# Indra-jith/failure-aware-vision

Hardware: AMD Instinct MI355X
Metric: frames/sec, ResNet-50 MC-Dropout T=30 224x224 batch=256 (higher is better)
Workload: dtype bf16; 1 GPU; BASELINE configs[2]: ResNet-50 v1.5 + MC-Dropout T=30 (all_blocks, p=0.10), 224x224x3 fp32 frames with Gaussian noise severity 3, batch 256 per GPU, synthetic frames and seeded synthetic weights; frames_per_gpu=256, global_batch=256, mc_samples=30, dropout_policy=all_blocks, inputs=resident in HBM before the timed region (H2D excluded), parallelism=batch sharded, 1 process per GPU, all-gather of (label, confidence)

## Files before the change

### failure_aware_vision_amd/_lib.py

```python
from __future__ import annotations

import ctypes as C
import os

_HERE = os.path.dirname(os.path.abspath(__file__))
LIB_PATH = os.environ.get("FAV_LIB_PATH") or os.path.join(_HERE, "lib", "libfav_hip.so")

FAV_OK = 0
STATUS_NAMES = {0: "FAV_OK", 1: "FAV_ERR_INVALID_ARG", 2: "FAV_ERR_BAD_BLOB", 3: "FAV_ERR_NO_WEIGHTS",
                4: "FAV_ERR_HIP", 5: "FAV_ERR_NO_DEVICE", 6: "FAV_ERR_UNSUPPORTED"}
LAYOUT_NHWC_U8, LAYOUT_NHWC_F32 = 0, 1
ARCH_RESNET18_CIFAR, ARCH_RESNET50, ARCH_VIT_B16, ARCH_VIT_TINY = 0, 1, 2, 3
CONF_MAX_SOFTMAX, CONF_ENTROPY, CONF_MUTUAL_INFO = 0, 1, 2
MATH_BF16, MATH_F32_EXACT = 0, 1
K_STEM, K_CONV, K_MAXPOOL, K_AVGPOOL, K_DROPOUT, K_HEAD, K_COUNT = 0, 1, 2, 3, 4, 5, 6
KERNEL_CLASS_NAMES = ("stem_im2col", "conv_igemm", "maxpool", "avgpool", "entry_dropout", "head")


class FavConfig(C.Structure):
    _fields_ = [
        ("struct_size", C.c_uint32), ("device", C.c_int32), ("arch", C.c_int32), ("num_classes", C.c_int32),
        ("in_h", C.c_int32), ("in_w", C.c_int32), ("max_batch", C.c_int32),
        ("mean", C.c_float * 3), ("stdev", C.c_float * 3),
        ("n_samples", C.c_int32), ("site_mask", C.c_uint32), ("dropout_p", C.c_float), ("seed", C.c_uint64),
# ... 54 lines not shown


class FavProfile(C.Structure):
    _fields_ = [("ms", C.c_double * K_COUNT), ("flops", C.c_double * K_COUNT), ("bytes", C.c_double * K_COUNT),
                ("launches", C.c_int64 * K_COUNT)]


class FavOpProfile(C.Structure):
    _fields_ = [("op_index", C.c_int32), ("kind", C.c_int32), ("H", C.c_int32), ("W", C.c_int32), ("Cin", C.c_int32),
                ("Ho", C.c_int32), ("Wo", C.c_int32), ("Cout", C.c_int32), ("kh", C.c_int32), ("kw", C.c_int32),
                ("stride", C.c_int32), ("reserved", C.c_int32), ("ms", C.c_double), ("flops", C.c_double),
                ("bytes", C.c_double), ("launches", C.c_int64)]


_SIGNATURES = {
    "fav_abi_version": (C.c_int32, []),
    "fav_default_config": (None, [C.POINTER(FavConfig), C.c_int32]),
    "fav_create": (C.c_int, [C.POINTER(FavConfig), C.POINTER(C.c_void_p)]),
    "fav_load_weights": (C.c_int, [C.c_void_p, C.c_void_p, C.c_size_t]),
    "fav_load_member_weights": (C.c_int, [C.c_void_p, C.c_int32, C.c_void_p, C.c_size_t]),
    "fav_destroy": (None, [C.c_void_p]),
    "fav_check_blob": (C.c_int, [C.c_void_p, C.c_size_t, C.c_char_p, C.c_size_t]),
    "fav_plan_schedule": (C.c_int, [C.POINTER(FavConfig), C.c_int32, C.c_char_p, C.c_size_t]),
    "fav_last_error": (C.c_char_p, [C.c_void_p]),
    "fav_classify": (C.c_int, [C.c_void_p, C.c_void_p, C.c_int32, C.c_int32, C.c_void_p, C.c_void_p, C.c_void_p]),
    "fav_classify_ex": (C.c_int, [C.c_void_p, C.c_void_p, C.c_int32, C.c_int32, C.c_int64, C.c_void_p, C.c_void_p,
                                  C.c_void_p, C.c_void_p, C.c_void_p]),
    "fav_classify_records": (C.c_int, [C.c_void_p, C.c_void_p, C.c_int32, C.c_int32, C.c_int64, C.c_void_p, C.c_void_p,
                                      C.c_void_p, C.c_void_p]),
    "fav_classify_uncertainty": (C.c_int, [C.c_void_p, C.c_void_p, C.c_int32, C.c_int32, C.c_int64, C.c_void_p, C.c_void_p,
                                          C.c_void_p, C.c_void_p]),
    "fav_classify_sets": (C.c_int, [C.c_void_p, C.c_void_p, C.c_int32, C.c_int32, C.c_int64, C.POINTER(FavConformal),
                                    C.c_void_p, C.c_void_p, C.c_void_p, C.c_void_p]),
    "fav_conformal_scores": (C.c_int, [C.c_void_p, C.c_void_p, C.c_int32, C.c_int32, C.c_int64, C.POINTER(FavConformal),
                                       C.c_void_p, C.c_void_p, C.c_void_p]),
    "fav_classify_sweep": (C.c_int, [C.c_void_p, C.c_void_p, C.c_int32, C.c_int32, C.c_int64, C.c_void_p, C.POINTER(C.c_float),
                                     C.c_int32, C.c_void_p, C.c_void_p]),
    "fav_set_temperature": (C.c_int, [C.c_void_p, C.c_float]),
    "fav_set_tau": (C.c_int, [C.c_void_p, C.c_float]),
    "fav_classify_host": (C.c_int, [C.c_void_p, C.c_void_p, C.c_int32, C.c_int32, C.c_int64, C.c_void_p, C.c_void_p,
                                    C.c_void_p, C.c_void_p]),
    "fav_get_logits": (C.c_int, [C.c_void_p, C.c_void_p, C.POINTER(C.c_int32), C.POINTER(C.c_int32), C.c_void_p]),
    "fav_set_profiling": (C.c_int, [C.c_void_p, C.c_int32]),
    "fav_get_profile": (C.c_int, [C.c_void_p, C.POINTER(FavProfile), C.c_int32]),
    "fav_get_op_profile": (C.c_int, [C.c_void_p, C.POINTER(FavOpProfile), C.c_int32, C.POINTER(C.c_int32)]),
    "fav_op_conv2d": (C.c_int, [C.POINTER(FavConvDesc), C.c_void_p]),
    "fav_op_bottleneck_tail": (C.c_int, [C.POINTER(FavTailDesc), C.c_void_p]),
    "fav_op_linear_streamk": (C.c_int, [C.POINTER(FavLinearDesc), C.c_void_p]),
    "fav_op_stem_im2col": (C.c_int, [C.c_void_p, C.c_int32, C.c_int32, C.c_int32, C.c_int32, C.c_int32, C.c_int32,
                                     C.c_int32, C.c_int32, C.c_int32, C.POINTER(C.c_float), C.POINTER(C.c_float),
                                     C.c_void_p, C.c_void_p]),
    "fav_op_stem_pool": (C.c_int, [C.c_void_p, C.c_int32, C.c_int32, C.c_int32, C.c_int32, C.c_void_p, C.c_void_p, C.c_void_p, C.c_void_p, C.c_void_p, C.c_void_p]),
    "fav_op_maxpool3x3s2": (C.c_int, [C.c_void_p, C.c_void_p, C.c_int32, C.c_int32, C.c_int32, C.c_int32, C.c_void_p]),
    "fav_op_avgpool": (C.c_int, [C.c_void_p, C.c_void_p, C.c_int32, C.c_int32, C.c_int32, C.POINTER(FavDropoutDesc),
                                 C.c_void_p]),
    "fav_op_entry_dropout": (C.c_int, [C.c_void_p, C.c_void_p, C.c_int64, C.c_int32, C.POINTER(FavDropoutDesc),
                                       C.c_void_p]),
    "fav_op_entry_reduce": (C.c_int, [C.c_void_p, C.c_void_p, C.c_void_p, C.c_void_p, C.c_void_p, C.c_int32, C.c_int32, C.c_int32,
                                      C.c_int32, C.POINTER(FavDropoutDesc), C.c_void_p]),
    "fav_op_layernorm": (C.c_int, [C.c_void_p, C.c_int64, C.c_void_p, C.c_void_p, C.c_void_p, C.c_int64, C.c_int32, C.c_float,
                                   C.c_void_p]),
    "fav_op_attention": (C.c_int, [C.c_void_p, C.c_void_p, C.c_int32, C.c_int32, C.c_int32, C.c_int32, C.c_int32, C.c_void_p]),
    "fav_op_vit_assemble": (C.c_int, [C.c_void_p, C.c_void_p, C.c_void_p, C.c_int32, C.c_int32, C.c_int32, C.c_void_p]),
    "fav_op_head": (C.c_int, [C.c_void_p, C.c_int32, C.c_int32, C.c_int32, C.c_int32, C.c_float, C.c_int32, C.c_float,
                              C.c_void_p, C.c_void_p, C.c_void_p, C.c_void_p, C.c_void_p]),
    "fav_op_head_uncertainty": (C.c_int, [C.c_void_p, C.c_int32, C.c_int32, C.c_int32, C.c_int32, C.c_float, C.c_int32,
                                          C.c_float, C.c_void_p, C.c_void_p, C.c_void_p, C.c_void_p]),
    "fav_op_head_sets": (C.c_int, [C.c_void_p, C.c_int32, C.c_int32, C.c_int32, C.c_int32, C.c_float, C.c_int32, C.c_float,
                                   C.c_int64, C.POINTER(FavConformal), C.c_void_p, C.c_void_p, C.c_void_p, C.c_void_p,
                                   C.c_void_p, C.c_void_p]),
# ... 36 lines not shown
```

### failure_aware_vision_amd/csrc/fav.hip

```cpp
#include <hip/hip_runtime.h>

#include <algorithm>
#include <atomic>
#include <cmath>
#include <cstdarg>
#include <cstdio>
#include <cstdlib>
#include <cstring>
#include <string>
#include <vector>

#include "../../include/fav.h"
#include "fav_kernels.hpp"
#include "fav_plan.hpp"

using namespace fav_plan;

namespace {

thread_local std::string g_create_error;

std::string fmt(const char* f, ...) {
    char buf[512];
    va_list ap;
// ... 331 lines not shown
    } while (0)
#define FAV_LAUNCH_BIG(MODE_)                                                                                     \
    do {                                                                                                          \
        const int pp = (int)FAV_KNOB("FAV_CONV_PP", 1);                                                           \
        if (d.relu == 2) {                                                                                        \
            if (epi && pp && MODE_ == 0) hipLaunchKernelGGL((conv_igemm_kernel<256, 256, 64, 2, 0, 2, 0, 1, 1, true>), grid, dim3(512), 0, s, p); \
            else if (epi) hipLaunchKernelGGL((conv_igemm_kernel<256, 256, 64, 2, MODE_, 2, 0, 1, 0, true>), grid, dim3(512), 0, s, p);    \
            else hipLaunchKernelGGL((conv_igemm_kernel<256, 256, 64, 2, MODE_, 2, 0, 0, 0, true>), grid, dim3(512), 0, s, p);        \
        } else if (epi && pp && MODE_ == 0) hipLaunchKernelGGL((conv_igemm_kernel<256, 256, 64, 2, 0, 2, 0, 1, 1>), grid, dim3(512), 0, s, p); \
        else if (epi) hipLaunchKernelGGL((conv_igemm_kernel<256, 256, 64, 2, MODE_, 2, 0, 1>), grid, dim3(512), 0, s, p);    \
        else hipLaunchKernelGGL((conv_igemm_kernel<256, 256, 64, 2, MODE_, 2, 0, 0>), grid, dim3(512), 0, s, p);        \
    } while (0)
    if (big) {
        if (d.math_mode == FAV_MATH_BF16) FAV_LAUNCH_BIG(0); else FAV_LAUNCH_BIG(1);
    } else if (d.math_mode == FAV_MATH_BF16) FAV_LAUNCH_MODE(0); else FAV_LAUNCH_MODE(1);
#undef FAV_LAUNCH_BIG
#undef FAV_LAUNCH_MODE
#undef FAV_LAUNCH
    dbg_report(tiles, BM, BN, BK);
    return nullptr;
}


const char* launch_tail(fav_handle* h, const fav_tail_desc& d, const Group& G, hipStream_t s) {
    const bool has3x3 = d.wb != nullptr;
    const int nred = d.wa ? d.Nred : 0;
    TailGeom g;
    if (!tail_geometry(d.Cmid, nred, has3x3, d.W, &g)) return "bottleneck tail: unsupported shape";
    const long long M = (long long)d.n_frames * d.H * d.W;
    if (M <= 0 || M > 0x7fffffffLL) return "bottleneck tail: row count out of range";
    TailParams p;
    p.t1 = (const uint16_t*)d.x; p.wb = (const uint16_t*)d.wb; p.bias_b = d.bias_b;
    p.wc = (const uint16_t*)d.wc; p.bias_c = d.bias_c; p.res = (const uint16_t*)d.res; p.y = (uint16_t*)d.y;
    p.wa = (const uint16_t*)d.wa; p.bias_a = d.bias_a; p.t1n = (uint16_t*)d.t1n;
    p.H = d.H; p.W = d.W; p.HW = d.H * d.W; p.M = (int)M;
    p.in_W = d.W; p.in_HW = p.HW; p.in_stride = 1;
    p.rega_bytes = g.rega_bytes;
    p.bias_b_off = g.bias_b_off; p.bias_ca_off = g.bias_ca_off; p.wa_off0 = g.wa_off0; p.wa_off1 = g.wa_off1; p.zero_off = g.zero_off;
    p.drop = make_drop(&d.drop);
    p.div_hw = fastdiv_make((uint32_t)p.HW);
    p.div_w = fastdiv_make((uint32_t)d.W);
    if (p.drop.site >= 0 && (p.drop.v0 < 0 || p.drop.v0 + d.n_frames > 0x7fffffffLL)) return "bottleneck tail: virtual frame index out of range";
    p.g_t1 = G.x; p.g_res = G.res; p.g_y = G.y; p.g_t1n = G.y2;
    p.g_wb = G.wb; p.g_bb = G.bb; p.g_wc = G.w; p.g_bc = G.b; p.g_wa = G.wa; p.g_ba = G.ba;
    p.site_e = d.entry_site;
    p.rs_T = 0; p.rs_tps = 0;
    if (d.res_entry) {
        if (!(d.Cmid == 64 && nred == 64 && has3x3) || p.drop.site < 0 || d.entry_site < 0 || !d.res)
            return "bottleneck tail: res_entry needs Cmid = Nred = 64 with the 3x3 and both dropout sites";
        if ((double)p.drop.n_img * p.HW * 4.0 * d.Cmid * 2.0 >= 2147483647.0) return "bottleneck tail: cached tensor too large for 32-bit offsets";
    }
    const int cmid = d.Cmid, cout = 4 * cmid;
    const double flops = 2.0 * (double)M * ((has3x3 ? 9.0 * cmid * cmid : 0.0) + (double)cmid * cout + (double)cout * nred) * G.n;
    const double res_rows = d.res_entry ? (double)std::min<long long>(d.n_frames, p.drop.n_img) * p.HW : (double)M;
    const double bytes = 2.0 * ((double)M * (cmid + 1.0 * cout + nred) + res_rows * cout + (has3x3 ? 9.0 * cmid * cmid : 0.0) + (double)cmid * cout + (double)cout * nred) * G.n;
    Prof pr(h, s, FAV_K_CONV, flops, bytes);
    { const int lds_pad = (int)FAV_KNOB("FAV_TAIL_LDS_PAD", 0); if (g.lds_bytes + lds_pad <= 160 * 1024) g.lds_bytes += lds_pad; }
    const int bm = g.rp * g.nw;
    const long long nblocks = (M + bm - 1) / bm;
    dim3 grid((unsigned)nblocks, G.n);
    p.dbg = nullptr;
    const bool dbg_on = FAV_KNOB("FAV_CONV_DBG", 0) != 0;
    if (dbg_on && !h) { (void)hipMalloc((void**)&p.dbg, (size_t)nblocks * 128); (void)hipMemset(p.dbg, 0, (size_t)nblocks * 128); }
    auto dbg_report = [&]() {
        if (!p.dbg) return;
        (void)hipStreamSynchronize(s);
        std::vector<unsigned long long> t((size_t)nblocks * 16);
        (void)hipMemcpy(t.data(), p.dbg, t.size() * 8, hipMemcpyDeviceToHost);
        (void)hipFree(p.dbg);
        if (const char* dump = fav_knob_str("FAV_CONV_DBG_DUMP")) {
            if (FILE* f = fopen(dump, "ab")) { const long long hdr[2] = {nblocks, cmid * 1000 + nred}; fwrite(hdr, 8, 2, f); fwrite(t.data(), 8, t.size(), f); fclose(f); }
        }
        unsigned long long lo = ~0ull, hi = 0;
        double ph[5] = {0, 0, 0, 0, 0};
        double cy[5] = {0, 0, 0, 0, 0};
        double cz[3] = {0, 0, 0};
        for (long long i = 0; i < nblocks; ++i) {
            lo = std::min(lo, t[i * 16]); hi = std::max(hi, t[i * 16 + 5]);
// ... 16 lines not shown
        static DeviceFlags attr_set;                                                                                  \
        if (!attr_set.test_current()) {                                                                               \
            if (hipFuncSetAttribute((const void*)bottleneck_tail_kernel<CMID_, NRED_, H3_, NS_, NW_, WC2_>,           \
                                    hipFuncAttributeMaxDynamicSharedMemorySize, 160 * 1024) != hipSuccess)            \
                return "bottleneck tail: cannot reserve LDS";                                                         \
            attr_set.set_current();                                                                                   \
        }                                                                                                             \
        hipLaunchKernelGGL((bottleneck_tail_kernel<CMID_, NRED_, H3_, NS_, NW_, WC2_>), grid, dim3(NW_ * 64), g.lds_bytes, s, p, g.patch_bytes); \
        dbg_report();                                                                                                 \
        return nullptr;                                                                                               \
    } while (0)
#define FAV_TAIL_W(CMID_, NRED_, H3_, NS_, NW_) do { if (g.wc2) FAV_TAIL(CMID_, NRED_, H3_, NS_, NW_, true); else FAV_TAIL(CMID_, NRED_, H3_, NS_, NW_, false); } while (0)
#define FAV_TAIL_N(CMID_, NRED_, H3_, NS_) FAV_TAIL_W(CMID_, NRED_, H3_, NS_, 4)
    if (d.res_entry) {
        const bool sample_minor = FAV_KNOB("FAV_ENTRY_RES_ORDER", 1) != 0;
        const long long sample_rows = (long long)p.drop.n_img * p.HW;
        if (sample_minor && p.drop.v0 % p.drop.n_img == 0 && d.n_frames % p.drop.n_img == 0 && sample_rows % bm == 0) {
            p.rs_T = d.n_frames / p.drop.n_img;
            p.rs_tps = (int)(sample_rows / bm);
        }
        static DeviceFlags attr_set;
        auto k0 = bottleneck_tail_kernel<64, 64, true, 3, 4, false, 32, 0, true, true, true>;
        auto k1 = bottleneck_tail_kernel<64, 64, true, 3, 4, true, 32, 0, true, true, true>;
        if (!attr_set.test_current()) {
            if (hipFuncSetAttribute((const void*)k0, hipFuncAttributeMaxDynamicSharedMemorySize, 160 * 1024) != hipSuccess ||
                hipFuncSetAttribute((const void*)k1, hipFuncAttributeMaxDynamicSharedMemorySize, 160 * 1024) != hipSuccess)
                return "bottleneck tail: cannot reserve LDS";
            attr_set.set_current();
        }
        if (g.wc2) hipLaunchKernelGGL(k1, grid, dim3(256), g.lds_bytes, s, p, g.patch_bytes);
        else hipLaunchKernelGGL(k0, grid, dim3(256), g.lds_bytes, s, p, g.patch_bytes);
        dbg_report();
        return nullptr;
    }
    if (cmid == 64) {
        if (has3x3) { if (nred == 0) FAV_TAIL_N(64, 0, true, 3); if (nred == 64) FAV_TAIL_N(64, 64, true, 3); if (nred == 128) FAV_TAIL_N(64, 128, true, 3); }
        else { if (nred == 0) FAV_TAIL_N(64, 0, false, 3); if (nred == 64) FAV_TAIL_N(64, 64, false, 3); if (nred == 128) FAV_TAIL_N(64, 128, false, 3); }
    } else if (cmid == 128) {
        if (has3x3) { if (nred == 0) FAV_TAIL_W(128, 0, true, 2, 8); if (nred == 128) FAV_TAIL_W(128, 128, true, 2, 8); }
        else { if (nred == 0) FAV_TAIL_W(128, 0, false, 2, 8); if (nred == 128) FAV_TAIL_W(128, 128, false, 2, 8); }
    } else if (cmid == 512) {
        FAV_TAIL(512, 0, false, 2, 8, true);
    } else if (nred == 0 && has3x3) {
        FAV_TAIL(256, 0, true, 2, 8, true);
    } else if (nred == 0) {
        FAV_TAIL_W(256, 0, false, 2, 4);
// ... 487 lines not shown
                case OP_CONV: {
                    const LayerShape& L = h->plan.layers[o.layer];
                    fav_conv_desc d;
                    d.x = buf(o.in, o); d.w = LW(o.layer); d.bias = LB(o.layer); d.res = buf(o.res, o); d.y = buf(o.out, o);
                    d.n_frames = cn; d.H = o.H; d.W = o.W; d.Cin = o.C; d.Cout = L.cout;
                    const bool stem = (o.in == B_A1);
                    d.kh = stem ? 1 : L.kh; d.kw = stem ? 1 : L.kw; d.stride = stem ? 1 : L.stride; d.pad = stem ? 0 : L.pad;
                    d.relu = o.relu; d.out_f32 = o.out_f32; d.math_mode = c.math_mode;
                    d.drop = dd;
                    const int ldy = o.out_f32 ? L.cout_pad : L.cout;
                    if (const char* e = launch_conv(h, d, L.cout_pad, ldy, G, s)) { h->err = e; return FAV_ERR_INVALID_ARG; }
                    break;
                }
                case OP_TAIL: {
                    fav_tail_desc d;
                    memset(&d, 0, sizeof d);
                    d.x = buf(o.in, o);
                    if (o.layer >= 0) { d.wb = LW(o.layer); d.bias_b = LB(o.layer); }
                    d.wc = LW(o.layer_c); d.bias_c = LB(o.layer_c); d.res = buf(o.res, o); d.y = buf(o.out, o);
                    if (o.layer_a >= 0) { d.wa = LW(o.layer_a); d.bias_a = LB(o.layer_a); d.t1n = buf(o.out2, o); }
                    d.n_frames = cn; d.H = o.H; d.W = o.W; d.Cmid = o.C; d.Nred = o.Co2;
                    d.drop = dd;
                    if (o.res_entry) { d.res = pin_base; d.res_entry = 1; d.entry_site = h->plan.first_site; }
                    if (const char* e = launch_tail(h, d, G, s)) { h->err = e; return FAV_ERR_INVALID_ARG; }
                    break;
                }
                case OP_STEM_POOL:
                    if (const char* e = launch_stem_pool(h, buf(o.in, o), layout, cn, o.H, o.W, LW(o.layer), LB(o.layer), c.mean, istd,
                                                         buf(o.out, o), G, s)) { h->err = e; return FAV_ERR_INVALID_ARG; }
                    break;
                case OP_MAXPOOL:
                    launch_maxpool(h, buf(o.in, o), buf(o.out, o), cn, o.H, o.W, o.C, s);
                    break;
                case OP_AVGPOOL: {
                    DropParams dp = make_drop(&dd);
                    launch_avgpool(h, buf(o.in, o), buf(o.out, o), cn, o.H * o.W, o.C, dp, G, s);
                    break;
                }
                case OP_ENTRY_DROPOUT: {
                    DropParams dp = make_drop(&dd);
                    launch_entry_dropout(h, pin_base, buf(o.out, o), o.in_elems, cn, dp, s);
                    break;
                }
                case OP_ENTRY_REDUCE: {
                    DropParams dp = make_drop(&dd);
                    if (const char* e = launch_entry_reduce(h, pin_base, o.skip_y ? nullptr : buf(o.out, o), LW(o.layer_a), LB(o.layer_a), buf(o.out2, o), o.C, o.Co2,
                                                            o.H * o.W, cn, dp, s)) { h->err = e; return FAV_ERR_INVALID_ARG; }
// ... 166 lines not shown
    if (st != FAV_OK) { g_create_error = h->err; free_all(h); delete h; return st; }
    *out = h;
    return FAV_OK;
}

fav_status fav_plan_schedule(const fav_config* cfg, int32_t flags, char* out, size_t cap) {
    if (!cfg || !out || cap < 2 || cfg->struct_size != sizeof(fav_config) || cfg->arch < 0 || cfg->arch > 1) return FAV_ERR_INVALID_ARG;
    Plan P;
    std::string err;
    fav_status st = plan_resnet(*cfg, cfg->n_members > 1 ? cfg->n_members : 1, (flags & 1) != 0, &P, &err);
    if (st != FAV_OK) { snprintf(out, cap, "%s", err.c_str()); return st; }
    std::string txt;
    for (size_t pi = 0; pi < P.phases.size(); ++pi)
        for (int i = P.phases[pi].op_begin; i < P.phases[pi].op_end; ++i) {
            const Op& o = P.ops[i];
            txt += fmt("op %d kind=%d phase=%zu layer=%d lc=%d la=%d in=%d res=%d out=%d out2=%d site=%d relu=%d suffix=%d rese=%d skipy=%d esite=%d\n", i, (int)o.kind, pi,
                       o.layer, o.layer_c, o.layer_a, o.in, o.res, o.out, o.out2, o.site, o.relu, (int)P.phases[pi].suffix, o.res_entry, o.skip_y, P.first_site);
        }
    if (txt.size() + 1 > cap) return FAV_ERR_INVALID_ARG;
    memcpy(out, txt.c_str(), txt.size() + 1);
    return FAV_OK;
}

void fav_destroy(fav_handle* h) {
    if (!h) return;
    (void)hipSetDevice(h->cfg.device);
    (void)hipDeviceSynchronize();
    free_all(h);
    delete h;
}

fav_status fav_load_weights(fav_handle* h, const void* blob, size_t size) { return fav_load_member_weights(h, 0, blob, size); }

fav_status fav_check_blob(const void* blob, size_t size, char* err, size_t err_cap) {
    auto fail = [&](const std::string& m) {
        if (err && err_cap) { snprintf(err, err_cap, "%s", m.c_str()); }
        return FAV_ERR_BAD_BLOB;
    };
    if (err && err_cap) err[0] = 0;
    if (!blob || size < 32) return fail("blob too small");
    const uint8_t* p = (const uint8_t*)blob;
    uint32_t hdr[8];
    memcpy(hdr, p, 32);
    if (hdr[0] != 0x57564146u || hdr[1] != 1u) return fail("not a FAVW v1 blob");
    const size_t nl = hdr[4];
    if (nl == 0 || nl > 4096) return fail("implausible layer count");
// ... 370 lines not shown
    *n_out = (int32_t)h->op_prof.size();
    if (out) for (int i = 0; i < cap && i < (int)h->op_prof.size(); ++i) out[i] = h->op_prof[i];
    return FAV_OK;
}

static fav_status op_done(const char* e) {
    if (e) { g_create_error = e; return FAV_ERR_INVALID_ARG; }
    if (hipGetLastError() != hipSuccess) { g_create_error = "kernel launch failed"; return FAV_ERR_HIP; }
    return FAV_OK;
}

fav_status fav_op_conv2d(const fav_conv_desc* d, void* stream) {
    if (!d || !d->x || !d->w || !d->bias || !d->y) return op_done("fav_op_conv2d: null pointer");
    if (d->Cout % 64 != 0) return op_done("fav_op_conv2d: Cout must be a multiple of 64");
    return op_done(launch_conv(nullptr, *d, d->Cout, d->Cout, Group{}, (hipStream_t)stream));
}

fav_status fav_op_bottleneck_tail(const fav_tail_desc* d, void* stream) {
    if (!d || !d->x || !d->wc || !d->bias_c || !d->res || !d->y) return op_done("fav_op_bottleneck_tail: null pointer");
    if ((d->wb && !d->bias_b) || (d->wa && (!d->bias_a || !d->t1n))) return op_done("fav_op_bottleneck_tail: null pointer");
    return op_done(launch_tail(nullptr, *d, Group{}, (hipStream_t)stream));
}

fav_status fav_op_stem_im2col(const void* images, int32_t layout, int32_t n, int32_t H, int32_t W, int32_t kh, int32_t kw,
                              int32_t stride, int32_t pad, int32_t kpad, const float* mean3, const float* inv_std3,
                              void* out, void* stream) {
    if (!images || !out || !mean3 || !inv_std3 || kpad % 64 != 0 || kpad < kh * kw * 3) return op_done("fav_op_stem_im2col: bad argument");
    launch_stem(nullptr, images, layout, n, H, W, kh, kw, stride, pad, kpad, mean3, inv_std3, out, (hipStream_t)stream);
    return op_done(nullptr);
}

fav_status fav_op_stem_pool(const void* images, int32_t layout, int32_t n, int32_t H, int32_t W, const void* w, const float* bias,
                            const float* mean3, const float* inv_std3, void* out, void* stream) {
    if (!images || !w || !bias || !mean3 || !inv_std3 || !out) return op_done("fav_op_stem_pool: null argument");
    return op_done(launch_stem_pool(nullptr, images, layout, n, H, W, w, bias, mean3, inv_std3, out, Group{}, (hipStream_t)stream));
}

fav_status fav_op_maxpool3x3s2(const void* x, void* y, int32_t n, int32_t H, int32_t W, int32_t C, void* stream) {
    if (!x || !y || C % 8 != 0) return op_done("fav_op_maxpool3x3s2: bad argument");
    launch_maxpool(nullptr, x, y, n, H, W, C, (hipStream_t)stream);
    return op_done(nullptr);
}

fav_status fav_op_avgpool(const void* x, void* y, int32_t n, int32_t HW, int32_t C, const fav_dropout_desc* drop, void* stream) {
    if (!x || !y || C % 16 != 0 || HW < 1) return op_done("fav_op_avgpool: bad argument");
    launch_avgpool(nullptr, x, y, n, HW, C, make_drop(drop), Group{}, (hipStream_t)stream);
// ... 109 lines not shown
```

### failure_aware_vision_amd/csrc/fav_kernels.hpp

```cpp
#pragma once
#include <hip/hip_runtime.h>
#include <float.h>
#include <stdint.h>

#ifdef FAV_EXPERIMENTS
#define FAV_DBG(P) ((P).dbg)
#else
#define FAV_DBG(P) ((unsigned long long*)nullptr)
#endif

namespace fav {

typedef __attribute__((__vector_size__(8 * sizeof(__bf16)))) __bf16 bf16x8_t;
typedef __attribute__((__vector_size__(4 * sizeof(float)))) float f32x4_t;

__device__ __forceinline__ float bf16_bits_to_f32(uint32_t b) { return __uint_as_float(b << 16); }

__device__ __forceinline__ uint32_t f32_to_bf16_bits(float f) {
    uint32_t u = __float_as_uint(f);
    return (u + 0x7FFFu + ((u >> 16) & 1u)) >> 16;
}
typedef __bf16 bf16x2_t __attribute__((ext_vector_type(2)));
typedef float f32x2_t __attribute__((ext_vector_type(2)));
typedef uint32_t u32x4_t __attribute__((ext_vector_type(4)));
// ... 1175 lines not shown
        __syncthreads();
        if (tid == 0) FAV_DBG(p)[blockIdx.x * 4ull + 3] = wall_clock64();
    }
}

struct TailParams {
    const uint16_t* t1;
    const uint16_t* wb; const float* bias_b;
    const uint16_t* wc; const float* bias_c;
    const uint16_t* res;
    uint16_t* y;
    const uint16_t* wa; const float* bias_a;
    uint16_t* t1n;
    int H, W, HW, M;
    int in_W, in_HW, in_stride;
    int rega_bytes;
    int bias_b_off, bias_ca_off, wa_off0, wa_off1, zero_off;
    DropParams drop;
    FastDiv div_hw, div_w;
    unsigned long long* dbg;
    long long g_t1, g_res, g_y, g_t1n, g_wb, g_bb, g_wc, g_bc, g_wa, g_ba;
    int site_e;
    int rs_T, rs_tps;
};

__device__ __forceinline__ TailParams tail_group_params(const TailParams& q) {
    TailParams p = q;
    const long long g = blockIdx.y;
    p.t1 = (const uint16_t*)((const char*)q.t1 + g * q.g_t1);
    if (q.wb) { p.wb = (const uint16_t*)((const char*)q.wb + g * q.g_wb); p.bias_b = (const float*)((const char*)q.bias_b + g * q.g_bb); }
    p.wc = (const uint16_t*)((const char*)q.wc + g * q.g_wc);
    p.bias_c = (const float*)((const char*)q.bias_c + g * q.g_bc);
    if (q.res) p.res = (const uint16_t*)((const char*)q.res + g * q.g_res);
    p.y = (uint16_t*)((char*)q.y + g * q.g_y);
    if (q.wa) { p.wa = (const uint16_t*)((const char*)q.wa + g * q.g_wa); p.bias_a = (const float*)((const char*)q.bias_a + g * q.g_ba); }
    if (q.t1n) p.t1n = (uint16_t*)((char*)q.t1n + g * q.g_t1n);
    return p;
}

#define FAV_BAR()                                               \
    do {                                                        \
        asm volatile("s_waitcnt lgkmcnt(0)" ::: "memory");      \
        __builtin_amdgcn_s_barrier();                           \
        asm volatile("" ::: "memory");                          \
    } while (0)

__device__ __forceinline__ int tail_row_perm(int r) {
    const int g = r & ~63, a = (r >> 4) & 3, i = r & 15;
    return g + 16 * (i >> 2) + 4 * a + (i & 3);
}

template <int CPR>
__device__ __forceinline__ int tail_sw(int row) {
    return CPR == 8 ? (row & 7) : (CPR == 16 ? ((row & 7) | ((row & 1) << 3)) : (row & 15));
}

template <int CMID, int NRED, bool HAS3X3, int NS, int NW, bool WC2, int RP = 32, int COUT_ = 0, bool HAS_RES = true, bool RELU = true, bool RESE = false>
__global__ __launch_bounds__(NW * 64, 2) void bottleneck_tail_kernel(const TailParams p_launch, int patch_bytes) {
    const TailParams p = tail_group_params(p_launch);
    constexpr bool LINEST = NRED > 0 || (HAS3X3 && !(HAS3X3 && CMID == 256));
    constexpr int COUT = COUT_ > 0 ? COUT_ : 4 * CMID;
    static_assert(HAS_RES || (!HAS3X3 && NRED == 0), "only conv_c alone runs without a residual");
    constexpr int BM = RP * NW, NT = NW * 64;
    static_assert(RP == 32 || (RP == 16 && !HAS3X3), "rows per wave");
    constexpr int ROWB = CMID * 2;
    constexpr int CPR = ROWB / 16;
    constexpr int PROWS = 1024 / ROWB;
    constexpr int CB = CMID / 64;
    constexpr int NKT = 9 * CB;
    constexpr int TM = 4;
    constexpr int WN1 = 2;
    constexpr int TN1 = CMID / WN1 / 16;
    constexpr int SLOT = CMID * 128;
    constexpr int BR = SLOT / 1024 / NW;
    constexpr int NCHUNK = COUT / 64;
    constexpr int KS2 = CMID / 32;
    constexpr int TM2 = RP / 16;
    constexpr int G3 = NRED / 64;
    constexpr int WC_BYTES = 64 * ROWB;
    constexpr int WA_BYTES = NRED * 128;
    constexpr int WCN = (HAS3X3 && CMID == 256) ? 4 : (WC2 ? 2 : 1);
    constexpr int BARQ = WCN == 4 ? 2 : 1;
    constexpr int P2W = WCN * WC_BYTES + 2 * WA_BYTES;
    constexpr int RING = HAS3X3 ? NS * SLOT : 0;
// ... 344 lines not shown
#pragma unroll
            for (int ks = 0; ks < KS2; ++ks) {
                const u32x4_t v = __builtin_amdgcn_raw_buffer_load_b128(srd_a, (int)(roff + (ks * 4 + fq) * 16), 0, 0);
                t2f[b][ks] = make_uint4(v[0], v[1], v[2], v[3]);
            }
        }
        FAV_T_BIAS_TO_LDS(true, true);
        asm volatile("s_waitcnt vmcnt(0)" ::: "memory");
        __syncthreads();
    }
    if (FAV_DBG(p) && tid == 0) FAV_DBG(p)[blockIdx.x * 16ull + 3] = wall_clock64();

    const __amdgpu_buffer_rsrc_t srd_y =
        __builtin_amdgcn_make_buffer_rsrc((void*)(p.y + (long long)m0 * COUT), 0, rows_valid * COUT * 2, 0x00020000);
    u32x4_t rcur[TM2][2];
    uint32_t drop_v[TM2], drop_pix[TM2];
#pragma unroll
    for (int b = 0; b < TM2; ++b) {
        const uint32_t m = (uint32_t)(m0 + wave * RP + b * 16 + frow);
        const uint32_t vl = fastdiv(m, p.div_hw);
        drop_v[b] = (uint32_t)p.drop.v0 + vl;
        drop_pix[b] = m - vl * (uint32_t)p.HW;
    }
    constexpr int NA3 = NRED > 0 ? NRED / 16 : 1;
    f32x4_t acc3[NA3][TM2];
#pragma unroll
    for (int a = 0; a < NA3; ++a)
#pragma unroll
        for (int b = 0; b < TM2; ++b) acc3[a][b] = (f32x4_t){0.f, 0.f, 0.f, 0.f};

#pragma unroll
    for (int j = 0; j < NCHUNK; ++j) {
        const unsigned char* const wcb = regb + (j % WCN) * WC_BYTES;
        const unsigned char* const wab = tsm + (((j + 1) & 1) ? p.wa_off1 : p.wa_off0);
        if ((j == 1 || j == 2) && FAV_DBG(p) && tid == 0) FAV_DBG(p)[blockIdx.x * 16ull + (j == 1 ? 12 : 14)] = __builtin_amdgcn_s_memtime();
        if (HAS_RES) {
#pragma unroll
            for (int b = 0; b < TM2; ++b) {
                asm volatile("" : "+v"(rnext[b][0]), "+v"(rnext[b][1]));
                rcur[b][0] = rnext[b][0];
                rcur[b][1] = rnext[b][1];
            }
        }
        if (j == 1 && FAV_DBG(p) && tid == 0) { asm volatile("s_nop 0" :: "v"(rcur[TM2 - 1][1])); FAV_DBG(p)[blockIdx.x * 16ull + 13] = __builtin_amdgcn_s_memtime(); }
        if (j + 1 < NCHUNK) {
            if (BARQ == 2) {
// ... 78 lines not shown
                    }
                    if (p.drop.site >= 0) {
#pragma unroll
                        for (int k = 0; k < 8; ++k) v[k] = FAV_DROP_APPLY(v[k], draws, 8 * g + k, p.drop);
                    }
                    u32x4_t o = {pack_bf16x2(v[0], v[1]), pack_bf16x2(v[2], v[3]), pack_bf16x2(v[4], v[5]), pack_bf16x2(v[6], v[7])};
                    if (RELU) {
#pragma unroll
                        for (int k = 0; k < 4; ++k) o[k] = relu_bf16x2(o[k]);
                    }
                    if (!LINEST) __builtin_amdgcn_raw_buffer_store_b128(o, srd_y, (row * COUT + n + 8 * g) * 2, 0, 0);
                    if (LINEST) *(u32x4_t*)(ych + row * 128 + (((2 * fq + g) ^ (row & 7)) << 4)) = o;
                }
            }
        }
        if (j == 1 && FAV_DBG(p) && tid == 0) FAV_DBG(p)[blockIdx.x * 16ull + 8] = __builtin_amdgcn_s_memtime();
        if constexpr (LINEST) {
            asm volatile("s_waitcnt lgkmcnt(0)" ::: "memory");
            {
#pragma unroll
                for (int i = 0; i < TM2 * 2; ++i) {
                    const int row = wave * RP + i * 8 + (lane >> 3);
                    const u32x4_t o = *(const u32x4_t*)(ych + row * 128 + (((lane & 7) ^ (row & 7)) << 4));
                    __builtin_amdgcn_raw_buffer_store_b128(o, srd_y, (row * COUT + j * 64 + (lane & 7) * 8) * 2, 0, 0);
                }
            }
        }
        if constexpr (NRED > 0) {
#pragma unroll
            for (int ks = 0; ks < 2; ++ks) {
                uint4 fy[TM2];
#pragma unroll
                for (int b = 0; b < TM2; ++b) {
                    const int row = wave * RP + b * 16 + frow;
                    fy[b] = *(const uint4*)(ych + row * 128 + (((ks * 4 + fq) ^ (row & 7)) << 4));
                }
#pragma unroll
                for (int a = 0; a < NA3; ++a) {
                    const int row = a * 16 + frow;
                    union { uint4 u; bf16x8_t v; } ua;
                    ua.u = *(const uint4*)(wab + row * 128 + (((ks * 4 + fq) ^ (row & 7)) << 4));
#pragma unroll
                    for (int b = 0; b < TM2; ++b) {
                        union { uint4 u; bf16x8_t v; } ub;
                        ub.u = fy[b];
                        acc3[a][b] = __builtin_amdgcn_mfma_f32_16x16x32_bf16(ua.v, ub.v, acc3[a][b], 0, 0, 0);
                    }
// ... 1562 lines not shown
```

### failure_aware_vision_amd/csrc/fav_plan.hpp

```cpp
#pragma once

#include <algorithm>
#include <cmath>
#include <cstdint>
#include <cstdlib>
#include <initializer_list>
#include <string>
#include <vector>

#include "../../include/fav.h"

namespace fav_plan {

#ifdef FAV_EXPERIMENTS
inline long long fav_knob_read(const char* name, long long dflt) { const char* e = getenv(name); return e ? atoll(e) : dflt; }
#define FAV_KNOB(NAME, DFLT) ([] { static const long long v_ = fav_plan::fav_knob_read(NAME, (DFLT)); return v_; }())
#else
#define FAV_KNOB(NAME, DFLT) ((long long)(DFLT))
#endif

struct ArchDef {
    bool bottleneck;
    int depths[4];
    int planes[4];
// ... 8 lines not shown
const VitDef kVit[2] = {{768, 12, 12, 3072, 16}, {128, 2, 2, 256, 16}};

struct LayerShape {
    int cout, cin, kh, kw, stride, pad;
    int cout_pad, k;
};

enum OpKind { OP_STEM_IM2COL, OP_CONV, OP_MAXPOOL, OP_AVGPOOL, OP_ENTRY_DROPOUT, OP_TAIL, OP_ENTRY_REDUCE, OP_STEM_POOL };
enum BufId { B_INPUT = -1, B_PHASE_IN = -2, B_PHASE_OUT = -3, B_NONE = -4, B_A1 = 5 };

struct Op {
    OpKind kind;
    int layer = -1;
    int layer_c = -1, layer_a = -1;
    int in = B_NONE, out = B_NONE, res = B_NONE;
    int out2 = B_NONE;
    int Co2 = 0;
    int H = 0, W = 0, C = 0;
    int Ho = 0, Wo = 0, Co = 0;
    int relu = 0, out_f32 = 0;
    int site = -1;
    int res_entry = 0;
    int skip_y = 0;
    long long in_elems = 0, out_elems = 0;
};

struct Phase {
    int op_begin, op_end;
    bool suffix;
    long long in_elems, out_elems;
    int out_bytes_per_elem;
    bool low_res;
    int chunk;
};
const int kMaxPhases = 4;

struct Plan {
    std::vector<LayerShape> layers;
    std::vector<Op> ops;
    std::vector<Phase> phases;
    int nblocks = 0;
    int first_site = -1;
    int T_eff = 1;
    int cpad = 0;
    bool has_mc = false, stem_fused = false;
    int ntok = 0;
// ... 210 lines not shown
        ph_suffix = true; ph_src = B_NONE;
        Op o; o.kind = OP_ENTRY_DROPOUT; o.in = B_PHASE_IN; o.out = cur; o.site = P.first_site;
        o.in_elems = o.out_elems = (long long)H * W * C;
        if (fusable && entry_reduce_enabled() && !entry_alone && next_pl > 0 && entry_reduce_supported(C, next_pl, c.max_batch, (long long)H * W)) {
            o.kind = OP_ENTRY_REDUCE; o.layer_a = (int)P.layers.size(); o.out2 = pre_t1 = other({cur}); o.Co2 = next_pl;
            o.H = H; o.W = W; o.C = C; o.relu = 1;
            entry_reduce = (int)P.ops.size();
        }
        P.ops.push_back(o);
    }

    void pool_fc() {
        if (regroup == P.nblocks) low_res_from_here();
        emit(OP_AVGPOOL, -1, cur, other({cur}), H, W, C, 1, 1, C).site = site_at(P.nblocks);
        cur = P.ops.back().out; H = W = 1;
        if (P.first_site == P.nblocks) entry(0);
        const int lfc = add_layer(P, c.num_classes, C, 1, 1, 1, 0);
        P.cpad = P.layers[lfc].cout_pad;
        Op& o = conv(lfc, cur, other({cur}), B_NONE, 0, 1, 1);
        o.out_f32 = 1; o.out_elems = P.cpad;
        close_phase();
    }
};

inline fav_status plan_resnet(const fav_config& c, int n_members, bool no_fuse, Plan* out, std::string* err) {
    const ArchDef& A = kArch[c.arch];
    Plan P;
    const int sk = A.imagenet_stem ? 7 : 3, ss = A.imagenet_stem ? 2 : 1, sp = A.imagenet_stem ? 3 : 1;
    const int Hs = conv_out(c.in_h, sk, ss, sp), Ws = conv_out(c.in_w, sk, ss, sp);
    if (Hs < 1 || Ws < 1) { *err = "input too small"; return FAV_ERR_INVALID_ARG; }
    P.nblocks = A.depths[0] + A.depths[1] + A.depths[2] + A.depths[3];
    const uint32_t valid_mask = (P.nblocks + 1 >= 32) ? 0xFFFFFFFFu : ((1u << (P.nblocks + 1)) - 1);
    if (c.site_mask & ~valid_mask) { *err = "site_mask has bits beyond the pooled-feature site"; return FAV_ERR_INVALID_ARG; }
    P.has_mc = c.site_mask != 0 && std::lround((double)c.dropout_p * 256.0) > 0;
    P.T_eff = P.has_mc ? c.n_samples : 1;
    for (int s = 0; P.has_mc && P.first_site < 0; ++s)
        if (c.site_mask >> s & 1) P.first_site = s;
    P.stem_fused = A.imagenet_stem && c.math_mode == FAV_MATH_BF16 && c.stem_fused >= 0 && !no_fuse &&
                   conv_out(Hs, 3, 2, 1) >= 1 && conv_out(Ws, 3, 2, 1) >= 1;
    int regroup = std::min(c.regroup_block < 0 ? A.depths[0] + A.depths[1] : c.regroup_block, P.nblocks);
    const bool entry_alone = P.has_mc && regroup == P.first_site + 1;
    if (entry_alone) regroup = -1;
    const bool fusable = tail_enabled() && !no_fuse && c.math_mode == FAV_MATH_BF16;
    ResNetWalk w{c, A, P, fusable, will_group(c, n_members, P, c.max_batch) ? n_members : 1, regroup, entry_alone, c.in_h, c.in_w};
    w.stem();
    for (int st = 0, b = 0; st < 4; ++st)
        for (int bi = 0; bi < A.depths[st]; ++bi, ++b) {
            const int next_pl = bi + 1 < A.depths[st] ? A.planes[st] : (st < 3 ? A.planes[st + 1] : 0);
            w.block(b, A.planes[st], (bi == 0 && st > 0) ? 2 : 1, next_pl);
            if (b == P.first_site) w.entry(A.bottleneck ? next_pl : 0);
        }
    w.pool_fc();
    if (P.phases.size() > (size_t)kMaxPhases) { *err = "schedule has more phases than a lane holds"; return FAV_ERR_UNSUPPORTED; }
    *out = std::move(P);
    return FAV_OK;
}

inline fav_status plan_vit(const fav_config& c, Plan* out, std::string* err) {
    const VitDef& V = kVit[c.arch - 2];
    if (c.in_h % V.patch || c.in_w % V.patch) { *err = "ViT input must be a multiple of the patch size"; return FAV_ERR_INVALID_ARG; }
    Plan P;
    P.ntok = (c.in_h / V.patch) * (c.in_w / V.patch) + 1;
    if (P.ntok > 256) { *err = "ViT path supports at most 256 tokens"; return FAV_ERR_UNSUPPORTED; }
    if (c.site_mask != 0 && c.dropout_p > 0.f) { *err = "the ViT path has no dropout sites"; return FAV_ERR_UNSUPPORTED; }
    if (c.n_members > 1) { *err = "the ViT path has no ensemble mode"; return FAV_ERR_UNSUPPORTED; }
    auto lin = [&](int cout, int cin, int kh, int kw, int stride) { add_layer(P, cout, cin, kh, kw, stride, 0); };
    auto vec = [&](int len) { P.layers.push_back({len, 0, 0, 0, 0, 0, len, 0}); };
    lin(V.dim, 3, V.patch, V.patch, V.patch);
    vec(P.ntok * V.dim);
    for (int i = 0; i < V.depth; ++i) {
        vec(V.dim); lin(3 * V.dim, V.dim, 1, 1, 1); lin(V.dim, V.dim, 1, 1, 1);
        vec(V.dim); lin(V.mlp, V.dim, 1, 1, 1); lin(V.dim, V.mlp, 1, 1, 1);
    }
    vec(V.dim);
    lin(c.num_classes, V.dim, 1, 1, 1);
    P.cpad = P.layers.back().cout_pad;
// ... 6 lines not shown
```

### include/fav.h

```cpp
#ifndef FAV_H
#define FAV_H

#include <stddef.h>
#include <stdint.h>

#ifdef __cplusplus
extern "C" {
#endif

#define FAV_ABI_VERSION 2

typedef struct fav_handle fav_handle;

typedef enum fav_status {
    FAV_OK = 0,
    FAV_ERR_INVALID_ARG = 1,
    FAV_ERR_BAD_BLOB = 2,
    FAV_ERR_NO_WEIGHTS = 3,
    FAV_ERR_HIP = 4,
    FAV_ERR_NO_DEVICE = 5,
    FAV_ERR_UNSUPPORTED = 6
} fav_status;

typedef enum fav_layout { FAV_LAYOUT_NHWC_U8 = 0, FAV_LAYOUT_NHWC_F32 = 1 } fav_layout;
// ... 16 lines not shown
    uint64_t seed;
    float temperature;
    int32_t conf_kind;
    float tau;
    int32_t math_mode;
    int32_t chunk_a;
    int32_t chunk_b;
    int32_t regroup_block;
    int32_t n_members;
    int32_t tail_min_rows;
    int32_t ens_grouped_max;
    int32_t vit_streams;
    int32_t stem_fused;
} fav_config;

void fav_default_config(fav_config* cfg, int32_t arch);

fav_status fav_create(const fav_config* cfg, fav_handle** out);
fav_status fav_load_weights(fav_handle* h, const void* blob_host, size_t size);
fav_status fav_load_member_weights(fav_handle* h, int32_t member, const void* blob_host, size_t size);
void fav_destroy(fav_handle* h);
fav_status fav_check_blob(const void* blob_host, size_t size, char* err, size_t err_cap);
fav_status fav_plan_schedule(const fav_config* cfg, int32_t flags, char* out, size_t cap);
const char* fav_last_error(const fav_handle* h);
int32_t fav_abi_version(void);


fav_status fav_classify(fav_handle* h, const void* images_dev, int32_t n, int32_t layout,
                        int32_t* labels_dev, float* conf_dev, void* hip_stream);

fav_status fav_classify_ex(fav_handle* h, const void* images_dev, int32_t n, int32_t layout,
                           int64_t first_image_index, int32_t* labels_dev, float* conf_dev,
                           uint8_t* fail_dev, float* score_dev, void* hip_stream);

fav_status fav_classify_records(fav_handle* h, const void* images_dev, int32_t n, int32_t layout,
                                int64_t first_image_index, void* records_dev, uint8_t* fail_dev,
                                float* score_dev, void* hip_stream);

typedef struct fav_uncertainty {
    int32_t label; float confidence; float mean_prob; float prob_std;
    float pred_entropy; float expected_entropy; float mutual_info; float agreement;
    int32_t top_label[5]; float top_prob[5];
} fav_uncertainty;

fav_status fav_classify_uncertainty(fav_handle* h, const void* images_dev, int32_t n, int32_t layout,
                                    int64_t first_image_index, fav_uncertainty* records_dev,
// ... 69 lines not shown
    const void* w;
    const float* bias;
    const void* res;
    void* y;
    int32_t n_frames, H, W, Cin, Cout, kh, kw, stride, pad;
    int32_t relu, out_f32, math_mode;
    fav_dropout_desc drop;
} fav_conv_desc;
fav_status fav_op_conv2d(const fav_conv_desc* d, void* hip_stream);

typedef struct fav_tail_desc {
    const void* x;
    const void* wb; const float* bias_b;
    const void* wc; const float* bias_c;
    const void* res;
    void* y;
    const void* wa; const float* bias_a;
    void* t1n;
    int32_t n_frames, H, W, Cmid, Nred;
    fav_dropout_desc drop;
    int32_t res_entry, entry_site;
} fav_tail_desc;
fav_status fav_op_bottleneck_tail(const fav_tail_desc* d, void* hip_stream);
fav_status fav_op_stem_im2col(const void* images, int32_t layout, int32_t n, int32_t H, int32_t W,
                              int32_t kh, int32_t kw, int32_t stride, int32_t pad, int32_t kpad,
                              const float* mean3, const float* inv_std3, void* out, void* hip_stream);
fav_status fav_op_stem_pool(const void* images, int32_t layout, int32_t n, int32_t H, int32_t W, const void* w, const float* bias,
                            const float* mean3, const float* inv_std3, void* out, void* hip_stream);
fav_status fav_op_maxpool3x3s2(const void* x, void* y, int32_t n, int32_t H, int32_t W, int32_t C, void* hip_stream);
fav_status fav_op_avgpool(const void* x, void* y, int32_t n, int32_t HW, int32_t C,
                          const fav_dropout_desc* drop, void* hip_stream);
fav_status fav_op_entry_dropout(const void* x, void* out, int64_t elems_per_frame, int32_t n_out,
                                const fav_dropout_desc* drop, void* hip_stream);
fav_status fav_op_entry_reduce(const void* x, void* y, const void* wa, const float* bias_a, void* t1, int32_t C, int32_t Nred,
                               int32_t HW, int32_t n_out, const fav_dropout_desc* drop, void* hip_stream);
fav_status fav_op_head(const float* logits, int32_t T, int32_t n, int32_t num_classes, int32_t ld,
                       float temperature, int32_t conf_kind, float tau,
                       int32_t* labels, float* conf, uint8_t* fail, float* score, void* hip_stream);
fav_status fav_op_head_uncertainty(const float* logits, int32_t T, int32_t n, int32_t num_classes, int32_t ld,
                                   float temperature, int32_t conf_kind, float tau, fav_uncertainty* records,
                                   uint8_t* fail, float* score, void* hip_stream);

fav_status fav_op_head_sets(const float* logits, int32_t T, int32_t n, int32_t num_classes, int32_t ld,
                            float temperature, int32_t conf_kind, float tau, int64_t first_image_index,
                            const fav_conformal* cp, const int32_t* true_labels, float* true_scores,
                            fav_pred_set* records, uint8_t* fail, float* score, void* hip_stream);
// ... 40 lines not shown
```

Baseline: 3470 frames/s.

## Store only even-pixel rows of bottleneck tail output consumed solely by stride-2 1x1 projection

Adds a planner pass that marks bottleneck tails (Cmid 64, Nred 128) in suffix phases whose output Y is read only by stride-2 1x1 projection convs. For those tails the kernel writes Y rows only at even (y,x) pixels, sending the other rows out of bounds through the buffer store. This cuts the HBM write traffic for Y by roughly three quarters. It relies on the plan analysis being right: any other reader of that buffer would see stale data.

```diff
diff --git a/failure_aware_vision_amd/_lib.py b/failure_aware_vision_amd/_lib.py
--- a/failure_aware_vision_amd/_lib.py
+++ b/failure_aware_vision_amd/_lib.py
@@ -100,6 +100,7 @@
     "fav_destroy": (None, [C.c_void_p]),
     "fav_check_blob": (C.c_int, [C.c_void_p, C.c_size_t, C.c_char_p, C.c_size_t]),
     "fav_plan_schedule": (C.c_int, [C.POINTER(FavConfig), C.c_int32, C.c_char_p, C.c_size_t]),
+    "fav_plan_sparse_stores": (C.c_int, [C.POINTER(FavConfig), C.c_int32, C.POINTER(C.c_int32), C.c_int32, C.POINTER(C.c_int32)]),
     "fav_last_error": (C.c_char_p, [C.c_void_p]),
     "fav_classify": (C.c_int, [C.c_void_p, C.c_void_p, C.c_int32, C.c_int32, C.c_void_p, C.c_void_p, C.c_void_p]),
     "fav_classify_ex": (C.c_int, [C.c_void_p, C.c_void_p, C.c_int32, C.c_int32, C.c_int64, C.c_void_p, C.c_void_p,
@@ -124,6 +125,7 @@
     "fav_get_op_profile": (C.c_int, [C.c_void_p, C.POINTER(FavOpProfile), C.c_int32, C.POINTER(C.c_int32)]),
     "fav_op_conv2d": (C.c_int, [C.POINTER(FavConvDesc), C.c_void_p]),
     "fav_op_bottleneck_tail": (C.c_int, [C.POINTER(FavTailDesc), C.c_void_p]),
+    "fav_op_bottleneck_tail_sparse": (C.c_int, [C.POINTER(FavTailDesc), C.c_void_p]),
     "fav_op_linear_streamk": (C.c_int, [C.POINTER(FavLinearDesc), C.c_void_p]),
     "fav_op_stem_im2col": (C.c_int, [C.c_void_p, C.c_int32, C.c_int32, C.c_int32, C.c_int32, C.c_int32, C.c_int32,
                                      C.c_int32, C.c_int32, C.c_int32, C.POINTER(C.c_float), C.POINTER(C.c_float),
diff --git a/failure_aware_vision_amd/csrc/fav.hip b/failure_aware_vision_amd/csrc/fav.hip
--- a/failure_aware_vision_amd/csrc/fav.hip
+++ b/failure_aware_vision_amd/csrc/fav.hip
@@ -377,9 +377,12 @@
 }
 
 
-const char* launch_tail(fav_handle* h, const fav_tail_desc& d, const Group& G, hipStream_t s) {
+bool tail_sparse_supported(int cmid, int nred, bool has3x3, bool res_entry) { return cmid == 64 && nred == 128 && has3x3 && !res_entry; }
+
+const char* launch_tail(fav_handle* h, const fav_tail_desc& d, const Group& G, hipStream_t s, bool y_sparse = false) {
     const bool has3x3 = d.wb != nullptr;
     const int nred = d.wa ? d.Nred : 0;
+    if (y_sparse && !tail_sparse_supported(d.Cmid, nred, has3x3, d.res_entry != 0)) return "bottleneck tail: the sparse store needs Cmid = 64, Nred = 128 with the 3x3";
     TailGeom g;
     if (!tail_geometry(d.Cmid, nred, has3x3, d.W, &g)) return "bottleneck tail: unsupported shape";
     const long long M = (long long)d.n_frames * d.H * d.W;
@@ -400,6 +403,7 @@
     p.g_wb = G.wb; p.g_bb = G.bb; p.g_wc = G.w; p.g_bc = G.b; p.g_wa = G.wa; p.g_ba = G.ba;
     p.site_e = d.entry_site;
     p.rs_T = 0; p.rs_tps = 0;
+    p.y_sparse = y_sparse ? 1 : 0;
     if (d.res_entry) {
         if (!(d.Cmid == 64 && nred == 64 && has3x3) || p.drop.site < 0 || d.entry_site < 0 || !d.res)
             return "bottleneck tail: res_entry needs Cmid = Nred = 64 with the 3x3 and both dropout sites";
@@ -408,7 +412,8 @@
     const int cmid = d.Cmid, cout = 4 * cmid;
     const double flops = 2.0 * (double)M * ((has3x3 ? 9.0 * cmid * cmid : 0.0) + (double)cmid * cout + (double)cout * nred) * G.n;
     const double res_rows = d.res_entry ? (double)std::min<long long>(d.n_frames, p.drop.n_img) * p.HW : (double)M;
-    const double bytes = 2.0 * ((double)M * (cmid + 1.0 * cout + nred) + res_rows * cout + (has3x3 ? 9.0 * cmid * cmid : 0.0) + (double)cmid * cout + (double)cout * nred) * G.n;
+    const double y_rows = y_sparse ? (double)d.n_frames * ((d.H + 1) / 2) * ((d.W + 1) / 2) : (double)M;
+    const double bytes = 2.0 * ((double)M * (cmid + nred) + y_rows * cout + res_rows * cout + (has3x3 ? 9.0 * cmid * cmid : 0.0) + (double)cmid * cout + (double)cout * nred) * G.n;
     Prof pr(h, s, FAV_K_CONV, flops, bytes);
     { const int lds_pad = (int)FAV_KNOB("FAV_TAIL_LDS_PAD", 0); if (g.lds_bytes + lds_pad <= 160 * 1024) g.lds_bytes += lds_pad; }
     const int bm = g.rp * g.nw;
@@ -471,6 +476,21 @@
         static DeviceFlags attr_set;
         auto k0 = bottleneck_tail_kernel<64, 64, true, 3, 4, false, 32, 0, true, true, true>;
         auto k1 = bottleneck_tail_kernel<64, 64, true, 3, 4, true, 32, 0, true, true, true>;
+        if (!attr_set.test_current()) {
+            if (hipFuncSetAttribute((const void*)k0, hipFuncAttributeMaxDynamicSharedMemorySize, 160 * 1024) != hipSuccess ||
+                hipFuncSetAttribute((const void*)k1, hipFuncAttributeMaxDynamicSharedMemorySize, 160 * 1024) != hipSuccess)
+                return "bottleneck tail: cannot reserve LDS";
+            attr_set.set_current();
+        }
+        if (g.wc2) hipLaunchKernelGGL(k1, grid, dim3(256), g.lds_bytes, s, p, g.patch_bytes);
+        else hipLaunchKernelGGL(k0, grid, dim3(256), g.lds_bytes, s, p, g.patch_bytes);
+        dbg_report();
+        return nullptr;
+    }
+    if (y_sparse) {
+        static DeviceFlags attr_set;
+        auto k0 = bottleneck_tail_kernel<64, 128, true, 3, 4, false, 32, 0, true, true, false, true>;
+        auto k1 = bottleneck_tail_kernel<64, 128, true, 3, 4, true, 32, 0, true, true, false, true>;
         if (!attr_set.test_current()) {
             if (hipFuncSetAttribute((const void*)k0, hipFuncAttributeMaxDynamicSharedMemorySize, 160 * 1024) != hipSuccess ||
                 hipFuncSetAttribute((const void*)k1, hipFuncAttributeMaxDynamicSharedMemorySize, 160 * 1024) != hipSuccess)
@@ -1004,7 +1024,7 @@
                     d.n_frames = cn; d.H = o.H; d.W = o.W; d.Cmid = o.C; d.Nred = o.Co2;
                     d.drop = dd;
                     if (o.res_entry) { d.res = pin_base; d.res_entry = 1; d.entry_site = h->plan.first_site; }
-                    if (const char* e = launch_tail(h, d, G, s)) { h->err = e; return FAV_ERR_INVALID_ARG; }
+                    if (const char* e = launch_tail(h, d, G, s, o.y_sparse != 0)) { h->err = e; return FAV_ERR_INVALID_ARG; }
                     break;
                 }
                 case OP_STEM_POOL:
@@ -1217,6 +1237,19 @@
     return FAV_OK;
 }
 
+fav_status fav_plan_sparse_stores(const fav_config* cfg, int32_t flags, int32_t* ops_out, int32_t cap, int32_t* n_out) {
+    if (!cfg || !n_out || cap < 0 || (cap > 0 && !ops_out) || cfg->struct_size != sizeof(fav_config) || cfg->arch < 0 || cfg->arch > 1) return FAV_ERR_INVALID_ARG;
+    Plan P;
+    std::string err;
+    fav_status st = plan_resnet(*cfg, cfg->n_members > 1 ? cfg->n_members : 1, (flags & 1) != 0, &P, &err);
+    if (st != FAV_OK) return st;
+    int32_t n = 0;
+    for (size_t i = 0; i < P.ops.size(); ++i)
+        if (P.ops[i].y_sparse) { if (n < cap) ops_out[n] = (int32_t)i; ++n; }
+    *n_out = n;
+    return FAV_OK;
+}
+
 void fav_destroy(fav_handle* h) {
     if (!h) return;
     (void)hipSetDevice(h->cfg.device);
@@ -1633,6 +1666,12 @@
     return op_done(launch_tail(nullptr, *d, Group{}, (hipStream_t)stream));
 }
 
+fav_status fav_op_bottleneck_tail_sparse(const fav_tail_desc* d, void* stream) {
+    if (!d || !d->x || !d->wb || !d->bias_b || !d->wc || !d->bias_c || !d->res || !d->y || !d->wa || !d->bias_a || !d->t1n)
+        return op_done("fav_op_bottleneck_tail_sparse: null pointer");
+    return op_done(launch_tail(nullptr, *d, Group{}, (hipStream_t)stream, true));
+}
+
 fav_status fav_op_stem_im2col(const void* images, int32_t layout, int32_t n, int32_t H, int32_t W, int32_t kh, int32_t kw,
                               int32_t stride, int32_t pad, int32_t kpad, const float* mean3, const float* inv_std3,
                               void* out, void* stream) {
diff --git a/failure_aware_vision_amd/csrc/fav_kernels.hpp b/failure_aware_vision_amd/csrc/fav_kernels.hpp
--- a/failure_aware_vision_amd/csrc/fav_kernels.hpp
+++ b/failure_aware_vision_amd/csrc/fav_kernels.hpp
@@ -1221,6 +1221,7 @@
     long long g_t1, g_res, g_y, g_t1n, g_wb, g_bb, g_wc, g_bc, g_wa, g_ba;
     int site_e;
     int rs_T, rs_tps;
+    int y_sparse;
 };
 
 __device__ __forceinline__ TailParams tail_group_params(const TailParams& q) {
@@ -1254,11 +1255,13 @@
     return CPR == 8 ? (row & 7) : (CPR == 16 ? ((row & 7) | ((row & 1) << 3)) : (row & 15));
 }
 
-template <int CMID, int NRED, bool HAS3X3, int NS, int NW, bool WC2, int RP = 32, int COUT_ = 0, bool HAS_RES = true, bool RELU = true, bool RESE = false>
+template <int CMID, int NRED, bool HAS3X3, int NS, int NW, bool WC2, int RP = 32, int COUT_ = 0, bool HAS_RES = true, bool RELU = true, bool RESE = false,
+          bool YSP = false>
 __global__ __launch_bounds__(NW * 64, 2) void bottleneck_tail_kernel(const TailParams p_launch, int patch_bytes) {
     const TailParams p = tail_group_params(p_launch);
     constexpr bool LINEST = NRED > 0 || (HAS3X3 && !(HAS3X3 && CMID == 256));
     constexpr int COUT = COUT_ > 0 ? COUT_ : 4 * CMID;
+    static_assert(!YSP || LINEST, "the sparse Y store is a mode of the line-order store loop");
     static_assert(HAS_RES || (!HAS3X3 && NRED == 0), "only conv_c alone runs without a residual");
     constexpr int BM = RP * NW, NT = NW * 64;
     static_assert(RP == 32 || (RP == 16 && !HAS3X3), "rows per wave");
@@ -1649,6 +1652,18 @@
         drop_v[b] = (uint32_t)p.drop.v0 + vl;
         drop_pix[b] = m - vl * (uint32_t)p.HW;
     }
+    uint32_t ysp_off[YSP ? TM2 * 2 : 1];
+    (void)ysp_off;
+    if constexpr (YSP) {
+#pragma unroll
+        for (int i = 0; i < TM2 * 2; ++i) {
+            const int row = wave * RP + i * 8 + (lane >> 3);
+            const uint32_t m = (uint32_t)(m0 + row);
+            const uint32_t pix = m - fastdiv(m, p.div_hw) * (uint32_t)p.HW;
+            const uint32_t y = fastdiv(pix, p.div_w), x = pix - y * (uint32_t)W;
+            ysp_off[i] = ((y | x) & 1u) ? OOB : (uint32_t)(row * COUT * 2);
+        }
+    }
     constexpr int NA3 = NRED > 0 ? NRED / 16 : 1;
     f32x4_t acc3[NA3][TM2];
 #pragma unroll
@@ -1773,7 +1788,8 @@
                 for (int i = 0; i < TM2 * 2; ++i) {
                     const int row = wave * RP + i * 8 + (lane >> 3);
                     const u32x4_t o = *(const u32x4_t*)(ych + row * 128 + (((lane & 7) ^ (row & 7)) << 4));
-                    __builtin_amdgcn_raw_buffer_store_b128(o, srd_y, (row * COUT + j * 64 + (lane & 7) * 8) * 2, 0, 0);
+                    if constexpr (YSP) __builtin_amdgcn_raw_buffer_store_b128(o, srd_y, (int)(ysp_off[i] + (uint32_t)((j * 64 + (lane & 7) * 8) * 2)), 0, 0);
+                    else __builtin_amdgcn_raw_buffer_store_b128(o, srd_y, (row * COUT + j * 64 + (lane & 7) * 8) * 2, 0, 0);
                 }
             }
         }
diff --git a/failure_aware_vision_amd/csrc/fav_plan.hpp b/failure_aware_vision_amd/csrc/fav_plan.hpp
--- a/failure_aware_vision_amd/csrc/fav_plan.hpp
+++ b/failure_aware_vision_amd/csrc/fav_plan.hpp
@@ -54,6 +54,7 @@
     int site = -1;
     int res_entry = 0;
     int skip_y = 0;
+    int y_sparse = 0;
     long long in_elems = 0, out_elems = 0;
 };
 
@@ -310,6 +311,31 @@
         close_phase();
     }
 };
+
+inline bool tail_sparse_shape(const Op& o) { return o.kind == OP_TAIL && o.C == 64 && o.Co2 == 128 && o.layer >= 0 && !o.res_entry; }
+
+inline void mark_sparse_stores(Plan& P) {
+    for (const Phase& ph : P.phases) {
+        if (!ph.suffix) continue;
+        for (int k = ph.op_begin; k < ph.op_end; ++k) {
+            Op& t = P.ops[k];
+            if (!tail_sparse_shape(t) || t.out < 0 || t.out > 4) continue;
+            int readers = 0;
+            bool ok = true;
+            for (int r = k + 1; r < ph.op_end && ok; ++r) {
+                const Op& o = P.ops[r];
+                if (o.res == t.out) ok = false;
+                if (o.in == t.out) {
+                    const bool proj = o.kind == OP_CONV && o.layer >= 0 && P.layers[o.layer].kh == 1 && P.layers[o.layer].kw == 1 &&
+                                      P.layers[o.layer].stride == 2 && P.layers[o.layer].pad == 0;
+                    if (proj) ++readers; else ok = false;
+                }
+                if (o.out == t.out || o.out2 == t.out) break;
+            }
+            t.y_sparse = ok && readers > 0;
+        }
+    }
+}
 
 inline fav_status plan_resnet(const fav_config& c, int n_members, bool no_fuse, Plan* out, std::string* err) {
     const ArchDef& A = kArch[c.arch];
@@ -340,6 +366,7 @@
         }
     w.pool_fc();
     if (P.phases.size() > (size_t)kMaxPhases) { *err = "schedule has more phases than a lane holds"; return FAV_ERR_UNSUPPORTED; }
+    mark_sparse_stores(P);
     *out = std::move(P);
     return FAV_OK;
 }
diff --git a/include/fav.h b/include/fav.h
--- a/include/fav.h
+++ b/include/fav.h
@@ -62,6 +62,7 @@
 void fav_destroy(fav_handle* h);
 fav_status fav_check_blob(const void* blob_host, size_t size, char* err, size_t err_cap);
 fav_status fav_plan_schedule(const fav_config* cfg, int32_t flags, char* out, size_t cap);
+fav_status fav_plan_sparse_stores(const fav_config* cfg, int32_t flags, int32_t* ops_out, int32_t cap, int32_t* n_out);
 const char* fav_last_error(const fav_handle* h);
 int32_t fav_abi_version(void);
 
@@ -177,6 +178,7 @@
     int32_t res_entry, entry_site;
 } fav_tail_desc;
 fav_status fav_op_bottleneck_tail(const fav_tail_desc* d, void* hip_stream);
+fav_status fav_op_bottleneck_tail_sparse(const fav_tail_desc* d, void* hip_stream);
 fav_status fav_op_stem_im2col(const void* images, int32_t layout, int32_t n, int32_t H, int32_t W,
                               int32_t kh, int32_t kw, int32_t stride, int32_t pad, int32_t kpad,
                               const float* mean3, const float* inv_std3, void* out, void* hip_stream);
```

Result: no change. 3487 frames/s (median of 6 runs) (+0.5%).
